# evan-wes/nerf-sandbox

Measured on NVIDIA B200. Metric: train_rays_per_s, higher is better.
Workload: dtype bf16

## Files before the change

nerf_sandbox_b200/csrc/field_tc.cu:

```cuda
#include <cuda.h>
#include <cuda_bf16.h>
#include <cuda_fp16.h>
#include <cstdio>
#include <mutex>
#include "nsb_common.cuh"
#include "tc_ptx.cuh"

namespace nsb {
namespace tc {

constexpr int TILE_M = 128;
constexpr int kStageBytes = 16384;
constexpr int kStages = 4;
constexpr int kActBytes = TILE_M * 256 * 2;
constexpr int kGxBytes = TILE_M * 64 * 2;
constexpr int kSmemAct = 0;
constexpr int kSmemGx = 2 * kActBytes;
constexpr int kSmemRing = kSmemGx + 2 * kGxBytes;
constexpr int kSmemBar = kSmemRing + kStages * kStageBytes;
constexpr int kSmemBias = kSmemBar + 256;
constexpr int kSmemBytes = kSmemBias + 2048;
constexpr int kThreads = 384;
constexpr int kStages2 = 8;
constexpr int kStageBytes2 = kStageBytes / 2;
// ... 823 lines not shown
            tail[layer_bias_ofs(m) + n] = params[d.b_off + n];
    }
    if (m == 0) {
        float* tail = reinterpret_cast<float*>(out + kBiasOfs);
        const LayerDesc ds = layer_desc(9), dc = layer_desc(11);
        for (int i = blockIdx.x * blockDim.x + threadIdx.x; i < 256; i += gridDim.x * blockDim.x) tail[kWsigOfs + i] = params[ds.w_off + i];
        for (int i = blockIdx.x * blockDim.x + threadIdx.x; i < 384; i += gridDim.x * blockDim.x) tail[kWoOfs + i] = params[dc.w_off + i];
        if (blockIdx.x == 0 && threadIdx.x < 4) {
            tail[kBsigOfs + threadIdx.x] = threadIdx.x == 0 ? params[ds.b_off] : 0.f;
            tail[kBoOfs + threadIdx.x] = threadIdx.x < 3 ? params[dc.b_off + threadIdx.x] : 0.f;
        }
    }
}

struct DgradParams {
    const float* d_raw;
    const uint8_t* packed;
    const uint8_t* stash;
    uint8_t* dstash;
    int64_t Q; int64_t num_tiles;
    alignas(64) CUtensorMap tm8;
};

__device__ __forceinline__ uint4 ldg16(const uint8_t* p) { return __ldg(reinterpret_cast<const uint4*>(p)); }
__device__ __forceinline__ float bf16lo(uint32_t w) { return __uint_as_float(w << 16); }
__device__ __forceinline__ float bf16hi(uint32_t w) { return __uint_as_float(w & 0xffff0000u); }

template <int KIND>
__device__ __forceinline__ void dgrad_chunk16(const uint32_t (&v)[16], int c0, uint32_t act, int r, float dsig, float hw0, uint32_t bits16) {
    uint32_t w[8];
#pragma unroll
    for (int j = 0; j < 8; ++j) {
        float a = __uint_as_float(v[2 * j]), b = __uint_as_float(v[2 * j + 1]);
        if (KIND == 1) {
            a = fmaf(dsig, __shfl_sync(0xffffffffu, hw0, (c0 & 16) + 2 * j), a);
            b = fmaf(dsig, __shfl_sync(0xffffffffu, hw0, (c0 & 16) + 2 * j + 1), b);
        }
        w[j] = pack_bf16(a, b);
        if (KIND != 0) w[j] &= relu_mask_word(bits16, j);
    }
    st_chunk(act, (c0 >> 3), r, w[0], w[1], w[2], w[3]);
    st_chunk(act, (c0 >> 3) + 1, r, w[4], w[5], w[6], w[7]);
}
template <int KIND>
__device__ __forceinline__ void dgrad_columns(uint32_t tmem_row, uint32_t act, int r, int lane, const float* __restrict__ tail,
                                              const uint4& mlo, const uint4& mhi, float dsig) {
    float hw0 = KIND == 1 ? __ldg(tail + kWsigOfs + lane) : 0.f;
    const uint32_t mw[8] = {mlo.x, mlo.y, mlo.z, mlo.w, mhi.x, mhi.y, mhi.z, mhi.w};
    uint32_t va[16], vb[16];
    tc_ld16(tmem_row, va);
#pragma unroll
    for (int i = 0; i < 8; ++i) {
        const int c0 = 32 * i;
        float n0 = 0.f;
        if (KIND == 1 && i < 7) n0 = __ldg(tail + kWsigOfs + c0 + 32 + lane);
        tc_wait_ld();
        tc_ld16(tmem_row + (uint32_t)c0 + 16u, vb);
        pin16(va);
        dgrad_chunk16<KIND>(va, c0, act, r, dsig, hw0, mw[i]);
        tc_wait_ld();
        tc_ld16(tmem_row + (uint32_t)(i < 7 ? c0 + 32 : c0), va);
        pin16(vb);
        dgrad_chunk16<KIND>(vb, c0 + 16, act, r, dsig, hw0, mw[i] >> 8);
        hw0 = n0;
    }
}

constexpr int kDgStages = 12;
constexpr int kDgSmemRing = kSmemGx;
static_assert(kDgSmemRing + kDgStages * kStageBytes2 == kSmemBar, "dgrad ring must end at the barrier block");
static_assert(kSmemBar + 8 * (3 * kDgStages + 6) + 4 <= kSmemBytes, "barrier block overflow");
__global__ void __cluster_dims__(2, 1, 1) __launch_bounds__(kThreads, 1) field_dgrad_kernel(const __grid_constant__ DgradParams p) {
    extern __shared__ __align__(128) uint8_t smem[];
    const uint32_t sbase = smem_u32(smem);
    const int warp = threadIdx.x >> 5, lane = threadIdx.x & 31;
    const uint32_t crank = cluster_ctarank();
    const uint32_t bar_full = sbase + kSmemBar, bar_empty = bar_full + 8 * kDgStages, bar_in = bar_empty + 8 * kDgStages,
                   bar_acc = bar_in + 16, bar_pfull = bar_acc + 16, bar_pin = bar_pfull + 8 * kDgStages;
    volatile uint32_t* tmem_slot = reinterpret_cast<volatile uint32_t*>(smem + kSmemBar + 8 * (3 * kDgStages + 6));
    if (threadIdx.x == 0) {
        for (int s = 0; s < kDgStages; ++s) { mbar_init(bar_full + 8 * s, 1); mbar_init(bar_empty + 8 * s, 1); mbar_init(bar_pfull + 8 * s, 1); }
        for (int t = 0; t < 2; ++t) { mbar_init(bar_in + 8 * t, 1); mbar_init(bar_acc + 8 * t, 1); mbar_init(bar_pin + 8 * t, 1); }
        asm volatile("fence.mbarrier_init.release.cluster;" ::: "memory");
    }
    if (warp == 2) {
        asm volatile("tcgen05.alloc.cta_group::2.sync.aligned.shared::cta.b32 [%0], %1;" ::"r"(smem_u32((const void*)tmem_slot)),
                     "r"(kTmemCols)
                     : "memory");
        asm volatile("tcgen05.relinquish_alloc_permit.cta_group::2.sync.aligned;" ::: "memory");
    }
    tc_fence_before();
    __syncthreads();
    cluster_sync_all();
    tc_fence_after();
    const uint32_t tmem_base = *tmem_slot;
    const int64_t num_pairs = (p.num_tiles + 1) / 2;
    const int64_t first_pair = (int64_t)blockIdx.x - crank;
    const int64_t n_iter = first_pair < num_pairs ? (num_pairs - first_pair + gridDim.x - 1) / gridDim.x : 0;
    const float* tail = reinterpret_cast<const float*>(p.packed + kBiasOfs);

    if (warp == 0) {
        {
            uint32_t stage = 0, round = 0;
            for (int64_t it = 0, pair = blockIdx.x; it < n_iter; ++it, pair += gridDim.x) {
                for (int m = 0; m < kNumDgradLayers; ++m) {
                    const uint8_t* src = p.packed + dgrad_layer_ofs(m);
                    const int ns = m == 0 ? 4 : 8;
                    for (int s = 0; s < ns; ++s) {
                        mbar_wait(bar_empty + 8 * stage, (round & 1) ^ 1);
                        if (elect_one()) {
                            if (crank == 0) mbar_expect_tx(bar_full + 8 * stage, kStageBytes);
                            tma_load_rows_to_leader(sbase + kDgSmemRing + stage * kStageBytes2, &p.tm8,
                                                    (dgrad_layer_ofs(m) + (uint32_t)s * kStageBytes + crank * kStageBytes2) >> 8, bar_full + 8 * stage);
                        }
                        __syncwarp();
                        if (++stage == kDgStages) { stage = 0; ++round; }
                    }
                }
            }
        }
    } else if (warp == 1) {
        if (crank == 0 && elect_one()) {
            uint32_t stage = 0, round = 0, use = 0;
            const uint32_t idesc = make_idesc2(256, kFmtBF16, kFmtBF16);
            const uint64_t ahi = desc_hi(2048, 128), bhi = desc_hi(2048, 128);
            const uint32_t ring_lo = (sbase + kDgSmemRing) >> 4;
            for (int64_t it = 0; it < n_iter; ++it) {
                for (int m = 0; m < kNumDgradLayers; ++m, ++use) {
                    const int ns = m == 0 ? 4 : 8;
                    const uint32_t stage0 = stage, round0 = round;
                    for (int t = 0; t < 2; ++t) {
                        mbar_wait(bar_in + 8 * t, use & 1);
                        mbar_wait_cl(bar_pin + 8 * t, use & 1);
                        tc_fence_after();
                        if (t == 1) { stage = stage0; round = round0; }
                        const uint32_t d_tmem = tmem_base + (uint32_t)t * 256u;
                        uint32_t a_lo = (sbase + kSmemAct + t * kActBytes) >> 4;
                        for (int s = 0; s < ns; ++s, a_lo += 512u) {
                            if (t == 0) {
                                mbar_wait(bar_full + 8 * stage, round & 1);
                                tc_fence_after();
                            }
                            const uint32_t b_lo = ring_lo + stage * (kStageBytes2 >> 4);
                            tc_mma2(d_tmem, ahi | (uint64_t)a_lo, bhi | (uint64_t)b_lo, idesc, s > 0 ? 1u : 0u);
                            tc_mma2(d_tmem, ahi | (uint64_t)(a_lo + 256u), bhi | (uint64_t)(b_lo + 256u), idesc, 1u);
                            if (s == ns - 1) tc_commit2(bar_acc + 8 * t);
                            if (t == 1) tc_commit2(bar_empty + 8 * stage);
                            if (++stage == kDgStages) { stage = 0; ++round; }
                        }
                    }
                }
            }
        }
    } else if (warp == 2 || warp == 3) {
        const int t = warp - 2;
        const uint32_t act = sbase + kSmemAct + t * kActBytes;
        named_bar_arrive(1 + t, 160);
        for (int64_t it = 0, pair = blockIdx.x; it < n_iter; ++it, pair += gridDim.x) {
            const int64_t tile = pair * 2 + t;
            uint8_t* ds_tile = tile < p.num_tiles ? p.dstash + (size_t)tile * kDstashTile : nullptr;
            const bool last_pair = it + 1 == n_iter;
            for (int e = 0; e <= kNumDgradLayers; ++e) {
                handoff_wait(t);
                if (lane == 0) {
                    if (e < kNumDgradLayers) arrive_in(crank, bar_in, bar_pin, t);
                    if (ds_tile) {
                        bulk_s2g(ds_tile + (e == 0 ? dstash_ofs(9) : dstash_ofs(8 - (e - 1))), act, e == 0 ? 32768u : 65536u);
                        bulk_commit();
                        bulk_wait_read0();
                    }
                }
                __syncwarp();
                if (!(last_pair && e == kNumDgradLayers)) named_bar_arrive(1 + t, 160);
            }
        }
        if (lane == 0) bulk_wait_all0();
    } else if (warp >= 4) {
        const int t = (warp - 4) >> 2;
        const int r = (int)threadIdx.x - 128 - t * 128;
        const uint32_t act = sbase + kSmemAct + t * kActBytes;
        const uint32_t tmem_row = tmem_base + (uint32_t)t * 256u + ((uint32_t)((warp & 3) * 32) << 16);
        uint32_t use = 0;
        for (int64_t it = 0, pair = blockIdx.x; it < n_iter; ++it, pair += gridDim.x) {
            const int64_t tile = pair * 2 + t;
            const int64_t q = tile * TILE_M + r;
            const bool tile_ok = tile < p.num_tiles;
            const bool valid = tile_ok && q < p.Q;
            const uint8_t* st_tile = p.stash + (size_t)(tile_ok ? tile : 0) * kStashTile;
            const float4 d = valid ? __ldg(reinterpret_cast<const float4*>(p.d_raw) + q) : make_float4(0.f, 0.f, 0.f, 0.f);
            named_bar_sync(1 + t, 160);
            {
                const uint8_t* mrow = st_tile + kStashMask + (size_t)r * 32;
                const uint4 cbits = ldg16(mrow + 8 * 4096);
                const uint32_t cw[4] = {cbits.x, cbits.y, cbits.z, cbits.w};
#pragma unroll
                for (int g = 0; g < 4; ++g) {
                    const float w0 = __ldg(tail + kWoOfs + 32 * g + lane), w1 = __ldg(tail + kWoOfs + 128 + 32 * g + lane),
                                w2 = __ldg(tail + kWoOfs + 256 + 32 * g + lane);
#pragma unroll
                    for (int c8 = 0; c8 < 4; ++c8) {
                        const uint32_t bits16 = cw[g] >> (8 * (c8 >> 1));
                        uint32_t w[4];
#pragma unroll
                        for (int j2 = 0; j2 < 4; ++j2) {
                            const int s0 = c8 * 8 + 2 * j2;
                            const float ga = d.x * __shfl_sync(0xffffffffu, w0, s0) + d.y * __shfl_sync(0xffffffffu, w1, s0) +
                                             d.z * __shfl_sync(0xffffffffu, w2, s0);
                            const float gb = d.x * __shfl_sync(0xffffffffu, w0, s0 + 1) + d.y * __shfl_sync(0xffffffffu, w1, s0 + 1) +
                                             d.z * __shfl_sync(0xffffffffu, w2, s0 + 1);
                            w[j2] = pack_bf16(ga, gb) & relu_mask_word(bits16, 4 * (c8 & 1) + j2);
                        }
                        st_chunk(act, g * 4 + c8, r, w[0], w[1], w[2], w[3]);
                    }
                }
            }
            handoff_signal(t);
            for (int m = 0; m < kNumDgradLayers; ++m, ++use) {
                uint4 mlo = make_uint4(0, 0, 0, 0), mhi = mlo;
                if (m >= 1) {
                    const uint8_t* mrow = st_tile + kStashMask + (size_t)(8 - m) * 4096 + (size_t)r * 32;
                    mlo = ldg16(mrow); mhi = ldg16(mrow + 16);
                }
                mbar_wait(bar_acc + 8 * t, use & 1);
                tc_fence_after();
                named_bar_sync(1 + t, 160);
                if (m == 0) dgrad_columns<0>(tmem_row, act, r, lane, tail, mlo, mhi, d.w);
                else if (m == 1) dgrad_columns<1>(tmem_row, act, r, lane, tail, mlo, mhi, d.w);
                else dgrad_columns<2>(tmem_row, act, r, lane, tail, mlo, mhi, d.w);
                handoff_signal(t);
            }
        }
    }
    tc_fence_before();
    __syncthreads();
    cluster_sync_all();
    if (warp == 2) {
        tc_fence_after();
        asm volatile("tcgen05.dealloc.cta_group::2.sync.aligned.b32 %0, %1;" ::"r"(tmem_base), "r"(kTmemCols) : "memory");
    }
}

struct WgPiece { uint32_t ofs; uint32_t bytes; int from_stash; int dy_half; int head; };
struct WgGroup { int a_piece, b_piece, b_piece2, tmem_col, n; };
enum { HEAD_NONE = 0, HEAD_SIGMA = 1, HEAD_RGB = 2 };
struct WgradJob {
    int n_pieces; WgPiece pieces[4];
    int n_groups; WgGroup groups[4];
    int release_after[4];
    int halves, xcols;
    int64_t w_dst;
    int ldw;
    int ncols_valid;
    int64_t b_dst;
    int64_t head_w_dst, head_b_dst;
    int cta_begin, cta_count;
};
constexpr int kMaxJobs = 16;
struct WgradParams {
    const uint8_t* stash; const uint8_t* dstash; const float* d_raw; float* grads;
    int64_t num_tiles, Q; int num_jobs; int dbg;
    WgradJob jobs[kMaxJobs];
};
constexpr int kWgPiece = 32768;
constexpr int kWgSlots = 6;
constexpr int kWgSmemBar = kWgSlots * kWgPiece;
constexpr int kWgSmemBytes = kWgSmemBar + 256;
constexpr int kWgThreads = 256;

__device__ __forceinline__ uint32_t make_idesc_mn(int N) {
    return (1u << 4) | (kFmtBF16 << 7) | (kFmtBF16 << 10) | (1u << 15) | (1u << 16) | ((uint32_t)(N >> 3) << 17) | ((uint32_t)(TILE_M >> 4) << 24);
}

template <int KIND>
__device__ __forceinline__ void wg_colsum(const uint8_t* img, int nchunks, int w4, int lane, const float4 (&dr)[4], float (&a0)[4][8],
                                          float (&a1)[4][8], float (&a2)[4][8]) {
#pragma unroll
    for (int ii = 0; ii < 4; ++ii) {
        const int c8 = w4 + 4 * ii;
        if (c8 < nchunks) {
#pragma unroll
            for (int rg = 0; rg < 4; ++rg) {
                const uint4 v = *reinterpret_cast<const uint4*>(img + (size_t)c8 * 2048 + (size_t)(rg * 32 + lane) * 16);
                const float x[8] = {bf16lo(v.x), bf16hi(v.x), bf16lo(v.y), bf16hi(v.y), bf16lo(v.z), bf16hi(v.z), bf16lo(v.w), bf16hi(v.w)};
#pragma unroll
                for (int j = 0; j < 8; ++j) {
                    if (KIND == 0) a0[ii][j] += x[j];
                    else if (KIND == 1) a0[ii][j] = fmaf(dr[rg].w, x[j], a0[ii][j]);
                    else {
                        a0[ii][j] = fmaf(dr[rg].x, x[j], a0[ii][j]); a1[ii][j] = fmaf(dr[rg].y, x[j], a1[ii][j]);
                        a2[ii][j] = fmaf(dr[rg].z, x[j], a2[ii][j]);
                    }
                }
            }
        }
    }
}

__global__ void __launch_bounds__(kWgThreads, 1) field_wgrad_kernel(const __grid_constant__ WgradParams p) {
    extern __shared__ __align__(128) uint8_t smem[];
    const uint32_t sbase = smem_u32(smem);
    const int warp = threadIdx.x >> 5, lane = threadIdx.x & 31;
    const uint32_t bar_full = sbase + kWgSmemBar, bar_empty = bar_full + 8 * kWgSlots, bar_done = bar_empty + 8 * kWgSlots;
    volatile uint32_t* tmem_slot = reinterpret_cast<volatile uint32_t*>(smem + kWgSmemBar + 8 * (2 * kWgSlots + 2));
    int ji = 0;
    for (int j = 0; j < p.num_jobs; ++j)
        if ((int)blockIdx.x >= p.jobs[j].cta_begin && (int)blockIdx.x < p.jobs[j].cta_begin + p.jobs[j].cta_count) ji = j;
    const WgradJob& job = p.jobs[ji];
    const int part = (int)blockIdx.x - job.cta_begin;
    if (threadIdx.x == 0) {
        for (int s = 0; s < kWgSlots; ++s) { mbar_init(bar_full + 8 * s, 1); mbar_init(bar_empty + 8 * s, 1 + 4); }
        mbar_init(bar_done, 1);
        asm volatile("fence.mbarrier_init.release.cluster;" ::: "memory");
    }
    if (warp == 2) {
        asm volatile("tcgen05.alloc.cta_group::1.sync.aligned.shared::cta.b32 [%0], %1;" ::"r"(smem_u32((const void*)tmem_slot)),
                     "r"(kTmemCols)
                     : "memory");
        asm volatile("tcgen05.relinquish_alloc_permit.cta_group::1.sync.aligned;" ::: "memory");
    }
    tc_fence_before();
    __syncthreads();
    tc_fence_after();
    const uint32_t tmem_base = *tmem_slot;
    int64_t my_tiles = 0;
    for (int64_t tile = part; tile < p.num_tiles; tile += job.cta_count) ++my_tiles;

    if (warp == 0) {
        uint32_t slot = 0, round = 0;
        for (int64_t tile = part; tile < p.num_tiles; tile += job.cta_count) {
            for (int i = 0; i < job.n_pieces; ++i) {
                const WgPiece& pc = job.pieces[i];
                const int64_t pt = p.num_tiles - 1 - tile;
                const uint8_t* src = pc.from_stash ? p.stash + (size_t)pt * kStashTile + pc.ofs : p.dstash + (size_t)pt * kDstashTile + pc.ofs;
                mbar_wait(bar_empty + 8 * slot, (round & 1) ^ 1);
                if (elect_one()) {
                    mbar_expect_tx(bar_full + 8 * slot, pc.bytes);
                    bulk_g2s(sbase + slot * kWgPiece, src, pc.bytes, bar_full + 8 * slot);
                }
                __syncwarp();
                if (++slot == kWgSlots) { slot = 0; ++round; }
            }
        }
    } else if (warp == 1) {
        if (elect_one()) {
            uint32_t slot = 0, round = 0;
            const uint64_t mnhi = desc_hi(128, 2048);
            bool first = true;
            long long w_full = 0; const long long t_begin = clock64();
            for (int64_t tile = part; tile < p.num_tiles; tile += job.cta_count) {
                uint32_t pslot[4], pround[4];
                for (int i = 0; i < job.n_pieces; ++i) { pslot[i] = slot; pround[i] = round; if (++slot == kWgSlots) { slot = 0; ++round; } }
                uint32_t ready = 0;
                for (int g = 0; g < job.n_groups; ++g) {
                    const WgGroup& gr = job.groups[g];
                    const long long tw0 = clock64();
                    if (!(ready >> gr.a_piece & 1)) { mbar_wait(bar_full + 8 * pslot[gr.a_piece], pround[gr.a_piece] & 1); ready |= 1u << gr.a_piece; }
                    if (!(ready >> gr.b_piece & 1)) { mbar_wait(bar_full + 8 * pslot[gr.b_piece], pround[gr.b_piece] & 1); ready |= 1u << gr.b_piece; }
                    if (gr.b_piece2 >= 0 && !(ready >> gr.b_piece2 & 1)) {
                        mbar_wait(bar_full + 8 * pslot[gr.b_piece2], pround[gr.b_piece2] & 1); ready |= 1u << gr.b_piece2;
                    }
                    w_full += clock64() - tw0;
                    tc_fence_after();
                    const uint32_t a_lo = (sbase + pslot[gr.a_piece] * kWgPiece) >> 4, b_lo = (sbase + pslot[gr.b_piece] * kWgPiece) >> 4;
                    const uint32_t idesc = make_idesc_mn(gr.n);
#pragma unroll
                    for (int ks = 0; ks < 8; ++ks)
                        tc_mma(tmem_base + (uint32_t)gr.tmem_col, mnhi | (uint64_t)(a_lo + ks * 16), mnhi | (uint64_t)(b_lo + ks * 16), idesc,
                               (!first || ks > 0) ? 1u : 0u);
                    for (int i = 0; i < job.n_pieces; ++i)
                        if (job.release_after[i] == g) tc_commit(bar_empty + 8 * pslot[i]);
                }
                for (int i = 0; i < job.n_pieces; ++i)
                    if (job.release_after[i] < 0) { mbar_wait(bar_full + 8 * pslot[i], pround[i] & 1); mbar_arrive(bar_empty + 8 * pslot[i]); }
                first = false;
            }
            tc_commit(bar_done);
            if (p.dbg && (part == 0)) printf("wgrad job %d (%d CTAs, %lld tiles): mma thread waited for pieces %lld of %lld cycles\n", ji, job.cta_count, (long long)my_tiles, w_full, clock64() - t_begin);
        }
    } else if (warp >= 4) {
        const int w4 = warp - 4;
        float bsum[2][4][8];
        float hacc[3][4][8];
        float dsum[4] = {0.f, 0.f, 0.f, 0.f};
#pragma unroll
        for (int i = 0; i < 4; ++i)
#pragma unroll
            for (int j = 0; j < 8; ++j) { bsum[0][i][j] = bsum[1][i][j] = 0.f; hacc[0][i][j] = hacc[1][i][j] = hacc[2][i][j] = 0.f; }
        const bool want_bias = job.b_dst >= 0;
        int job_head = HEAD_NONE;
        for (int i = 0; i < job.n_pieces; ++i) if (job.pieces[i].head) job_head = job.pieces[i].head;
        auto load_dr = [&](int64_t tile, float4 (&dr)[4]) {
#pragma unroll
            for (int rg = 0; rg < 4; ++rg) {
                const int64_t q = (p.num_tiles - 1 - tile) * TILE_M + rg * 32 + lane;
                dr[rg] = (tile < p.num_tiles && q < p.Q) ? __ldg(reinterpret_cast<const float4*>(p.d_raw) + q) : make_float4(0.f, 0.f, 0.f, 0.f);
            }
        };
        {
            uint32_t slot = 0, round = 0;
            float4 dr[4], dr_next[4];
            if (job_head) load_dr(part, dr_next);
            for (int64_t tile = part; tile < p.num_tiles; tile += job.cta_count) {
                if (job_head) {
#pragma unroll
                    for (int rg = 0; rg < 4; ++rg) dr[rg] = dr_next[rg];
                    load_dr(tile + job.cta_count, dr_next);
                    if (w4 == 0) {
#pragma unroll
                        for (int rg = 0; rg < 4; ++rg) { dsum[0] += dr[rg].x; dsum[1] += dr[rg].y; dsum[2] += dr[rg].z; dsum[3] += dr[rg].w; }
                    }
                }
                int xhalf = 0;
                for (int i = 0; i < job.n_pieces; ++i) {
                    const WgPiece& pc = job.pieces[i];
                    mbar_wait(bar_full + 8 * slot, round & 1);
                    const uint8_t* img = smem + slot * kWgPiece;
                    const int nchunks = (int)(pc.bytes >> 11);
                    if (pc.dy_half == 0 && want_bias) wg_colsum<0>(img, nchunks, w4, lane, dr, bsum[0], bsum[0], bsum[0]);
                    else if (pc.dy_half == 1 && want_bias) wg_colsum<0>(img, nchunks, w4, lane, dr, bsum[1], bsum[1], bsum[1]);
                    if (pc.head == HEAD_SIGMA) {
                        if (xhalf == 0) wg_colsum<1>(img, nchunks, w4, lane, dr, hacc[0], hacc[0], hacc[0]);
                        else wg_colsum<1>(img, nchunks, w4, lane, dr, hacc[1], hacc[1], hacc[1]);
                        ++xhalf;
                    } else if (pc.head == HEAD_RGB) {
                        wg_colsum<2>(img, nchunks, w4, lane, dr, hacc[0], hacc[1], hacc[2]);
                    }
                    __syncwarp();
                    if (lane == 0) mbar_arrive(bar_empty + 8 * slot);
                    if (++slot == kWgSlots) { slot = 0; ++round; }
                }
            }
        }
        if (my_tiles > 0) {
            if (want_bias) {
#pragma unroll
                for (int a = 0; a < 2; ++a)
#pragma unroll
                    for (int ii = 0; ii < 4; ++ii)
#pragma unroll
                        for (int j = 0; j < 8; ++j) {
                            const float sum = warp_sum(bsum[a][ii][j]);
                            if (lane == 0 && a < job.halves) atomicAdd(p.grads + job.b_dst + a * 128 + (w4 + 4 * ii) * 8 + j, sum);
                        }
            }
            if (job_head == HEAD_SIGMA) {
#pragma unroll
                for (int a = 0; a < 2; ++a)
#pragma unroll
                    for (int ii = 0; ii < 4; ++ii)
#pragma unroll
                        for (int j = 0; j < 8; ++j) {
                            const float sum = warp_sum(hacc[a][ii][j]);
                            if (lane == 0) atomicAdd(p.grads + job.head_w_dst + a * 128 + (w4 + 4 * ii) * 8 + j, sum);
                        }
                if (w4 == 0) { const float sd = warp_sum(dsum[3]); if (lane == 0) atomicAdd(p.grads + job.head_b_dst, sd); }
            } else if (job_head == HEAD_RGB) {
#pragma unroll
                for (int ch = 0; ch < 3; ++ch)
#pragma unroll
                    for (int ii = 0; ii < 4; ++ii)
#pragma unroll
                        for (int j = 0; j < 8; ++j) {
                            const float sum = warp_sum(hacc[ch][ii][j]);
                            if (lane == 0) atomicAdd(p.grads + job.head_w_dst + ch * 128 + (w4 + 4 * ii) * 8 + j, sum);
                        }
                if (w4 == 0) {
                    const float a0 = warp_sum(dsum[0]), a1 = warp_sum(dsum[1]), a2 = warp_sum(dsum[2]);
                    if (lane == 0) { atomicAdd(p.grads + job.head_b_dst, a0); atomicAdd(p.grads + job.head_b_dst + 1, a1); atomicAdd(p.grads + job.head_b_dst + 2, a2); }
                }
            }
            if (job.n_groups > 0) {
                mbar_wait(bar_done, 0);
                tc_fence_after();
                for (int h = 0; h < job.halves; ++h) {
                    const int n = h * 128 + w4 * 32 + lane;
                    const uint32_t trow = tmem_base + (uint32_t)h * 256u + ((uint32_t)(w4 * 32) << 16);
                    for (int c0 = 0; c0 < job.xcols; c0 += 32) {
                        uint32_t v[32];
                        tc_ld32(trow + (uint32_t)c0, v);
                        tc_wait_ld();
                        float* dst = p.grads + job.w_dst + (int64_t)n * job.ldw + c0;
#pragma unroll
                        for (int j = 0; j < 32; ++j)
                            if (c0 + j < job.ncols_valid) atomicAdd(dst + j, __uint_as_float(v[j]));
                    }
                }
            }
        }
    }
    tc_fence_before();
    __syncthreads();
    if (warp == 2) {
        tc_fence_after();
        asm volatile("tcgen05.dealloc.cta_group::1.sync.aligned.b32 %0, %1;" ::"r"(tmem_base), "r"(kTmemCols) : "memory");
    }
}

struct DinputParams {
    const uint8_t* packed; const uint8_t* dstash;
    float* d_enc_pos; float* d_enc_dir;
    int64_t Q, num_tiles;
};
constexpr int kDiSlab = 16384;
constexpr int kDiStages = 4;
constexpr int kDiSlabs = 10;
constexpr int kDiSmemRing = kDinImgBytes;
constexpr int kDiSmemOut = kDiSmemRing + kDiStages * kDiSlab;
constexpr int kDiOutFloats = TILE_M * (kPosDim + kDirDim);
constexpr int kDiSmemBar = kDiSmemOut + kDiOutFloats * 4;
constexpr int kDiSmemBytes = kDiSmemBar + 256;
constexpr int kDiThreads = 256;
constexpr uint32_t kDiTmemCols = 256;
static_assert(kDiSmemBytes <= 227 * 1024, "dinput shared memory");
__host__ __device__ inline size_t dinput_slab_ofs(int s) {
    return s < 4 ? dstash_ofs(0) + (size_t)s * kDiSlab : (s < 8 ? dstash_ofs(4) + (size_t)(s - 4) * kDiSlab : dstash_ofs(9) + (size_t)(s - 8) * kDiSlab);
}

__global__ void __launch_bounds__(kDiThreads, 1) field_dinput_kernel(const __grid_constant__ DinputParams p) {
    extern __shared__ __align__(128) uint8_t smem[];
    const uint32_t sbase = smem_u32(smem);
    const int warp = threadIdx.x >> 5;
    const uint32_t bar_full = sbase + kDiSmemBar, bar_empty = bar_full + 8 * kDiStages, bar_acc = bar_empty + 8 * kDiStages,
                   bar_free = bar_acc + 16, bar_b = bar_free + 16;
    volatile uint32_t* tmem_slot = reinterpret_cast<volatile uint32_t*>(smem + kDiSmemBar + 8 * (2 * kDiStages + 5));
    if (threadIdx.x == 0) {
        for (int s = 0; s < kDiStages; ++s) { mbar_init(bar_full + 8 * s, 1); mbar_init(bar_empty + 8 * s, 1); }
        for (int a = 0; a < 2; ++a) { mbar_init(bar_acc + 8 * a, 1); mbar_init(bar_free + 8 * a, 128); }
        mbar_init(bar_b, 1);
        asm volatile("fence.mbarrier_init.release.cluster;" ::: "memory");
    }
    if (warp == 2) {
        asm volatile("tcgen05.alloc.cta_group::1.sync.aligned.shared::cta.b32 [%0], %1;" ::"r"(smem_u32((const void*)tmem_slot)),
                     "r"(kDiTmemCols)
                     : "memory");
        asm volatile("tcgen05.relinquish_alloc_permit.cta_group::1.sync.aligned;" ::: "memory");
    }
    tc_fence_before();
    __syncthreads();
    tc_fence_after();
    const uint32_t tmem_base = *tmem_slot;

    if (warp == 0) {
        if (elect_one()) {
            mbar_expect_tx(bar_b, kDinImgBytes);
            bulk_g2s(sbase, p.packed + kDinImgOfs, kDinImgBytes, bar_b);
            uint32_t stage = 0, round = 0;
            for (int64_t tile = blockIdx.x; tile < p.num_tiles; tile += gridDim.x) {
                const uint8_t* ds = p.dstash + (size_t)tile * kDstashTile;
                for (int s = 0; s < kDiSlabs; ++s) {
                    mbar_wait(bar_empty + 8 * stage, (round & 1) ^ 1);
                    mbar_expect_tx(bar_full + 8 * stage, kDiSlab);
                    bulk_g2s(sbase + kDiSmemRing + stage * kDiSlab, ds + dinput_slab_ofs(s), kDiSlab, bar_full + 8 * stage);
                    if (++stage == kDiStages) { stage = 0; ++round; }
                }
            }
        }
    } else if (warp == 1) {
        if (elect_one()) {
            constexpr uint32_t idesc_base = (1u << 4) | (1u << 7) | (1u << 10) | ((uint32_t)(TILE_M >> 4) << 24);
            constexpr uint32_t idesc_x = idesc_base | ((uint32_t)(64 >> 3) << 17), idesc_d = idesc_base | ((uint32_t)(32 >> 3) << 17);
            const uint64_t ahi = desc_hi(2048, 128), bhi_x = desc_hi(64 * 16, 128), bhi_d = desc_hi(32 * 16, 128);
            mbar_wait(bar_b, 0);
            uint32_t stage = 0, round = 0, it = 0;
            for (int64_t tile = blockIdx.x; tile < p.num_tiles; tile += gridDim.x, ++it) {
                const uint32_t acc = it & 1;
                mbar_wait(bar_free + 8 * acc, ((it >> 1) & 1) ^ 1);
                tc_fence_after();
                const uint32_t d_x = tmem_base + acc * 128, d_d = d_x + 64;
                for (int s = 0; s < kDiSlabs; ++s) {
                    mbar_wait(bar_full + 8 * stage, round & 1);
                    tc_fence_after();
                    const uint32_t a0 = sbase + kDiSmemRing + stage * kDiSlab;
#pragma unroll
                    for (int j = 0; j < 4; ++j) {
                        const uint64_t ad = desc_at(ahi, a0 + j * 4096);
                        if (s < 8) {
                            const uint32_t k0 = (uint32_t)(s & 3) * 64 + j * 16;
                            const uint32_t b = sbase + (s < 4 ? kDinPos0 : kDinPos4) + (k0 >> 3) * 1024;
                            tc_mma(d_x, ad, desc_at(bhi_x, b), idesc_x, (s == 0 && j == 0) ? 0u : 1u);
                        } else {
                            const uint32_t k0 = (uint32_t)(s - 8) * 64 + j * 16;
                            tc_mma(d_d, ad, desc_at(bhi_d, sbase + kDinDir + (k0 >> 3) * 512), idesc_d, (s == 8 && j == 0) ? 0u : 1u);
                        }
                    }
                    tc_commit(bar_empty + 8 * stage);
                    if (++stage == kDiStages) { stage = 0; ++round; }
                }
                tc_commit(bar_acc + 8 * acc);
            }
        }
    } else if (warp >= 4) {
        const int r = (int)threadIdx.x - 128;
        float* out_x = reinterpret_cast<float*>(smem + kDiSmemOut);
        float* out_d = out_x + TILE_M * kPosDim;
        uint32_t it = 0;
        for (int64_t tile = blockIdx.x; tile < p.num_tiles; tile += gridDim.x, ++it) {
            const uint32_t acc = it & 1;
            mbar_wait(bar_acc + 8 * acc, (it >> 1) & 1);
            tc_fence_after();
            const uint32_t trow = tmem_base + acc * 128 + ((uint32_t)((warp & 3) * 32) << 16);
#pragma unroll 1
            for (int c = 0; c < 6; ++c) {
                uint32_t v[16];
                tc_ld16(trow + 16 * c, v);
                tc_wait_ld();
                pin16(v);
#pragma unroll
                for (int j = 0; j < 16; ++j) {
                    const int col = 16 * c + j;
                    if (col < kPosDim) out_x[r * kPosDim + col] = __uint_as_float(v[j]);
                    else if (col >= 64 && col < 64 + kDirDim) out_d[r * kDirDim + col - 64] = __uint_as_float(v[j]);
                }
            }
            tc_fence_before();
            mbar_arrive(bar_free + 8 * acc);
            named_bar_sync(1, 128);
            const int64_t rows = p.Q - tile * TILE_M < TILE_M ? p.Q - tile * TILE_M : TILE_M;
            if (p.d_enc_pos) {
                float* dst = p.d_enc_pos + tile * TILE_M * kPosDim;
                for (int i = r; i < rows * kPosDim; i += 128) dst[i] = out_x[i];
            }
            if (p.d_enc_dir) {
                float* dst = p.d_enc_dir + tile * TILE_M * kDirDim;
                for (int i = r; i < rows * kDirDim; i += 128) dst[i] = out_d[i];
            }
            named_bar_sync(1, 128);
        }
    }
    tc_fence_before();
    __syncthreads();
    if (warp == 2) {
        tc_fence_after();
        asm volatile("tcgen05.dealloc.cta_group::1.sync.aligned.b32 %0, %1;" ::"r"(tmem_base), "r"(kDiTmemCols) : "memory");
    }
}

__device__ __forceinline__ void pack_tc_dinput(const float* __restrict__ params, uint8_t* __restrict__ out) {
    const LayerDesc d0 = layer_desc(0), d4 = layer_desc(4), dc = layer_desc(10);
    for (int idx = blockIdx.x * blockDim.x + threadIdx.x; idx < 2 * 32 * 64 + 16 * 32; idx += gridDim.x * blockDim.x) {
        int img = idx >> 11, rem = idx & 2047;
        if (img > 2) img = 2;
        if (img == 2) rem = idx - 2 * 2048;
        const int rows = img < 2 ? 64 : 32, n = rem % rows, k8 = rem / rows;
        const LayerDesc& d = img == 0 ? d0 : (img == 1 ? d4 : dc);
        const int col = img == 0 ? n : kHidden + n, n_true = img < 2 ? kPosDim : kDirDim;
        float x[8];
#pragma unroll
        for (int j = 0; j < 8; ++j) x[j] = n < n_true ? params[d.w_off + (int64_t)(8 * k8 + j) * d.K + col] : 0.f;
        const uint32_t base = img == 0 ? kDinPos0 : (img == 1 ? kDinPos4 : kDinDir);
        *reinterpret_cast<uint4*>(out + kDinImgOfs + base + (size_t)(k8 * rows + n) * 16) =
            make_uint4(pack_bf16(x[0], x[1]), pack_bf16(x[2], x[3]), pack_bf16(x[4], x[5]), pack_bf16(x[6], x[7]));
    }
}

__device__ __forceinline__ void pack_tc_transposed(const float* __restrict__ params, uint8_t* __restrict__ out, int m) {
    {
        const int pl = m == 0 ? 10 : (m == 1 ? 8 : 9 - m);
        const LayerDesc d = layer_desc(pl);
        const int Nout = d.N;
        __nv_bfloat16* img = reinterpret_cast<__nv_bfloat16*>(out + dgrad_layer_ofs(m));
        for (int idx = blockIdx.x * blockDim.x + threadIdx.x; idx < (Nout >> 3) * 256; idx += gridDim.x * blockDim.x) {
            const int n8 = idx >> 8, j = idx & 255;
            const float* col = params + d.w_off + (int64_t)(8 * n8) * d.K + j;
            uint32_t w[4];
#pragma unroll
            for (int q = 0; q < 4; ++q) w[q] = pack_bf16(col[(int64_t)(2 * q) * d.K], col[(int64_t)(2 * q + 1) * d.K]);
            reinterpret_cast<uint4*>(img)[(((size_t)(n8 >> 2) * 2 + (j >> 7)) * 4 + (n8 & 3)) * 128 + (j & 127)] = make_uint4(w[0], w[1], w[2], w[3]);
        }
    }
}
struct PackBatch { const float* params[4]; uint8_t* out[4]; uint64_t* counter; };
__global__ void pack_tc_kernel(const PackBatch b) {
    if (b.counter && blockIdx.x == 0 && blockIdx.y == 0 && blockIdx.z == 0 && threadIdx.x == 0) *b.counter += 1;
    const float* params = b.params[blockIdx.z];
    uint8_t* out = b.out[blockIdx.z];
    if (blockIdx.y < kNumMmaLayers) pack_tc_forward<0>(params, out, blockIdx.y);
    else if (blockIdx.y < kNumMmaLayers + kNumDgradLayers) pack_tc_transposed(params, out, blockIdx.y - kNumMmaLayers);
    else if (blockIdx.y == kNumMmaLayers + kNumDgradLayers) pack_tc_dinput(params, out);
    else if (blockIdx.y < 2 * kNumMmaLayers + kNumDgradLayers + 1) pack_tc_forward<1>(params, out, blockIdx.y - kNumMmaLayers - kNumDgradLayers - 1);
    else pack_tc_forward<2>(params, out, blockIdx.y - 2 * kNumMmaLayers - kNumDgradLayers - 1);
}

}

size_t tc_packed_bytes() { return align_up(tc::kPackedTcBytes, 256); }

size_t tc_workspace_bytes(int64_t Q, int stash) {
    const int64_t tiles = cdiv(Q, tc::TILE_M);
    return 256 + (stash ? (size_t)tiles * (tc::kStashTile + tc::kDstashTile) : 0);
}
size_t tc_stash_tile_bytes() { return tc::kStashTile; }
static inline uint8_t* ws_stash(void* ws) { return reinterpret_cast<uint8_t*>(ws) + 256; }
static inline uint8_t* ws_dstash(void* ws, int64_t Q) { return ws_stash(ws) + (size_t)cdiv(Q, tc::TILE_M) * tc::kStashTile; }

int tc_pack(const float* const* params, void* const* packed_bf16, int n_nets, bool train_only, cudaStream_t st) {
    tc::PackBatch b{};
    for (int i = 0; i < n_nets; ++i) { b.params[i] = params[i]; b.out[i] = reinterpret_cast<uint8_t*>(packed_bf16[i]); }
    b.counter = g_pack_counter;
    const int ny = train_only ? tc::kNumMmaLayers + tc::kNumDgradLayers + 1 : 3 * tc::kNumMmaLayers + tc::kNumDgradLayers + 1;
    tc::pack_tc_kernel<<<dim3(32, ny, n_nets), 256, 0, st>>>(b);
    NSB_LAUNCH_CHECK("pack_tc_kernel");
    return NSB_OK;
}

int check_arch() {
    static int ok = -1;
    if (ok < 0) {
        int dev = 0, major = 0;
        cudaGetDevice(&dev);
        cudaDeviceGetAttribute(&major, cudaDevAttrComputeCapabilityMajor, dev);
        ok = major == 10 ? 1 : 0;
    }
    return ok ? NSB_OK : NSB_E_ARCH;
}

struct PackedMaps { const void* ptr; CUtensorMap tm8, tm4; };
static int packed_maps(const void* packed, CUtensorMap* tm8, CUtensorMap* tm4) {
    typedef CUresult (*EncodeFn)(CUtensorMap*, CUtensorMapDataType, cuuint32_t, void*, const cuuint64_t*, const cuuint64_t*, const cuuint32_t*,
                                 const cuuint32_t*, CUtensorMapInterleave, CUtensorMapSwizzle, CUtensorMapL2promotion, CUtensorMapFloatOOBfill);
    static std::mutex mu;
    static EncodeFn encode = nullptr;
    static PackedMaps cache[16];
    static int n_cached = 0, next = 0;
    std::lock_guard<std::mutex> lock(mu);
    for (int i = 0; i < n_cached; ++i)
        if (cache[i].ptr == packed) { *tm8 = cache[i].tm8; if (tm4) *tm4 = cache[i].tm4; return NSB_OK; }
    if (!encode) {
        void* fn = nullptr;
        cudaDriverEntryPointQueryResult q;
        if (cudaGetDriverEntryPoint("cuTensorMapEncodeTiled", &fn, cudaEnableDefault, &q) != cudaSuccess || !fn)
            return check_launch("cudaGetDriverEntryPoint(cuTensorMapEncodeTiled)");
        encode = reinterpret_cast<EncodeFn>(fn);
    }
    PackedMaps m{};
    m.ptr = packed;
    const cuuint64_t dims[2] = {256, tc::kPackedTcBytes / 256};
    const cuuint64_t strides[1] = {256};
    const cuuint32_t estr[2] = {1, 1};
    for (int k = 0; k < 2; ++k) {
        const cuuint32_t box[2] = {256, k == 0 ? 32u : 16u};
        if (encode(k == 0 ? &m.tm8 : &m.tm4, CU_TENSOR_MAP_DATA_TYPE_UINT8, 2, const_cast<void*>(packed), dims, strides, box, estr,
                   CU_TENSOR_MAP_INTERLEAVE_NONE, CU_TENSOR_MAP_SWIZZLE_NONE, CU_TENSOR_MAP_L2_PROMOTION_L2_256B,
                   CU_TENSOR_MAP_FLOAT_OOB_FILL_NONE) != CUDA_SUCCESS) {
            snprintf(g_cuda_err, sizeof(g_cuda_err), "cuTensorMapEncodeTiled failed for the packed weight buffer");
            return NSB_E_CUDA;
        }
    }
    cache[next] = m; next = (next + 1) % 16; if (n_cached < 16) ++n_cached;
    *tm8 = m.tm8; if (tm4) *tm4 = m.tm4;
    return NSB_OK;
}

template <bool FROM_ENC>
static int launch_fwd(tc::FwdParams& p, cudaStream_t st) {
    NSB_TRY(check_arch());
    static bool attr_set = false;
    if (!attr_set) {
        if (cudaFuncSetAttribute(tc::field_fwd_kernel<FROM_ENC, false>, cudaFuncAttributeMaxDynamicSharedMemorySize, tc::kSmemBytes) != cudaSuccess ||
            cudaFuncSetAttribute(tc::field_fwd_kernel<FROM_ENC, true>, cudaFuncAttributeMaxDynamicSharedMemorySize, tc::kSmemBytes) != cudaSuccess)
            return check_launch("cudaFuncSetAttribute(field_fwd_kernel)");
        attr_set = true;
    }
    p.num_tiles = cdiv(p.Q, tc::TILE_M);
    NSB_TRY(packed_maps(p.packed, &p.tm8, &p.tm4));
    const int64_t pairs = (p.num_tiles + 1) / 2;
    int grid = (int)(pairs < num_sms() ? pairs : num_sms());
    grid = (grid + 1) / 2 * 2;
    if (grid > num_sms()) grid -= 2;
    if (p.stash) tc::field_fwd_kernel<FROM_ENC, true><<<grid, tc::kThreads, tc::kSmemBytes, st>>>(p);
    else tc::field_fwd_kernel<FROM_ENC, false><<<grid, tc::kThreads, tc::kSmemBytes, st>>>(p);
    NSB_LAUNCH_CHECK("field_fwd_kernel");
    return NSB_OK;
}

template <bool FROM_ENC>
static int launch_fwd_split(tc::FwdParams& p, cudaStream_t st) {
    NSB_TRY(check_arch());
    static bool attr_set = false;
    if (!attr_set) {
        if (cudaFuncSetAttribute(tc::field_fwd_split_kernel<FROM_ENC>, cudaFuncAttributeMaxDynamicSharedMemorySize, tc::kSmemBytes) != cudaSuccess)
            return check_launch("cudaFuncSetAttribute(field_fwd_split_kernel)");
        attr_set = true;
    }
    p.num_tiles = cdiv(p.Q, tc::TILE_M);
    NSB_TRY(packed_maps(p.packed, &p.tm8, &p.tm4));
    const int64_t pairs = (p.num_tiles + 1) / 2;
    const int64_t max_pairs = num_sms() / 2;
    const int grid = 2 * (int)(pairs < max_pairs ? pairs : max_pairs);
    tc::field_fwd_split_kernel<FROM_ENC><<<grid, tc::kThreads, tc::kSmemBytes, st>>>(p);
    NSB_LAUNCH_CHECK("field_fwd_split_kernel");
    return NSB_OK;
}

int tc_field_fwd_rays_split(const float* rays_o, const float* rays_d, const float* z, const float* ray_norm, const float* viewdirs,
                            const void* packed, float* raw, int64_t B, int N, cudaStream_t st) {
    tc::FwdParams p{};
    p.rays_o = rays_o; p.rays_d = rays_d; p.z = z; p.ray_norm = ray_norm; p.viewdirs = viewdirs;
    p.packed = reinterpret_cast<const uint8_t*>(packed); p.raw = raw;
    p.Q = B * (int64_t)N; p.N = N;
    return launch_fwd_split<false>(p, st);
}
int tc_field_fwd_enc_split(const float* enc_pos, const float* enc_dir, const void* packed, float* raw, int64_t Q, cudaStream_t st) {
    tc::FwdParams p{};
    p.enc_pos = enc_pos; p.enc_dir = enc_dir;
    p.packed = reinterpret_cast<const uint8_t*>(packed); p.raw = raw;
    p.Q = Q; p.N = 1;
    return launch_fwd_split<true>(p, st);
}

int tc_field_fwd_rays(const float* rays_o, const float* rays_d, const float* z, const float* ray_norm, const float* viewdirs,
                      const void* packed, float* raw, void* ws, int64_t B, int N, int stash, cudaStream_t st) {
    tc::FwdParams p{};
    p.rays_o = rays_o; p.rays_d = rays_d; p.z = z; p.ray_norm = ray_norm; p.viewdirs = viewdirs;
    p.packed = reinterpret_cast<const uint8_t*>(packed); p.raw = raw;
    p.stash = stash ? ws_stash(ws) : nullptr;
    p.Q = B * (int64_t)N; p.N = N;
    return launch_fwd<false>(p, st);
}

int tc_field_fwd_enc(const float* enc_pos, const float* enc_dir, const void* packed, float* raw, void* ws, int64_t Q,
                     int stash, cudaStream_t st) {
    tc::FwdParams p{};
    p.enc_pos = enc_pos; p.enc_dir = enc_dir;
    p.packed = reinterpret_cast<const uint8_t*>(packed); p.raw = raw;
    p.stash = stash ? ws_stash(ws) : nullptr;
    p.Q = Q; p.N = 1;
    return launch_fwd<true>(p, st);
}

int tc_field_bwd(const float* d_raw, const void* packed, float* grads, float* d_enc_pos, float* d_enc_dir, void* ws, int64_t Q,
                 cudaStream_t st) {
    NSB_TRY(check_arch());
    static bool attr_set = false;
    if (!attr_set) {
        if (cudaFuncSetAttribute(tc::field_dgrad_kernel, cudaFuncAttributeMaxDynamicSharedMemorySize, tc::kSmemBytes) != cudaSuccess ||
            cudaFuncSetAttribute(tc::field_wgrad_kernel, cudaFuncAttributeMaxDynamicSharedMemorySize, tc::kWgSmemBytes) != cudaSuccess ||
            cudaFuncSetAttribute(tc::field_dinput_kernel, cudaFuncAttributeMaxDynamicSharedMemorySize, tc::kDiSmemBytes) != cudaSuccess)
            return check_launch("cudaFuncSetAttribute(bwd kernels)");
        attr_set = true;
    }
    const int64_t tiles = cdiv(Q, tc::TILE_M);
    const int64_t pairs = (tiles + 1) / 2;
    tc::DgradParams dp{};
    dp.d_raw = d_raw; dp.packed = reinterpret_cast<const uint8_t*>(packed); dp.stash = ws_stash(ws); dp.dstash = ws_dstash(ws, Q);
    dp.Q = Q; dp.num_tiles = tiles;
    NSB_TRY(packed_maps(packed, &dp.tm8, nullptr));
    int dgrid = (int)(pairs < num_sms() ? pairs : num_sms());
    dgrid = (dgrid + 1) / 2 * 2;
    if (dgrid > num_sms()) dgrid -= 2;
    tc::field_dgrad_kernel<<<dgrid, tc::kThreads, tc::kSmemBytes, st>>>(dp);
    NSB_LAUNCH_CHECK("field_dgrad_kernel");
    if (d_enc_pos || d_enc_dir) {
        tc::DinputParams ip{};
        ip.packed = reinterpret_cast<const uint8_t*>(packed); ip.dstash = ws_dstash(ws, Q);
        ip.d_enc_pos = d_enc_pos; ip.d_enc_dir = d_enc_dir; ip.Q = Q; ip.num_tiles = tiles;
        const int igrid = (int)(tiles < num_sms() ? tiles : num_sms());
        tc::field_dinput_kernel<<<igrid, tc::kDiThreads, tc::kDiSmemBytes, st>>>(ip);
        NSB_LAUNCH_CHECK("field_dinput_kernel");
    }
    if (!grads) return NSB_OK;

    tc::WgradParams wp{};
    wp.stash = ws_stash(ws); wp.dstash = ws_dstash(ws, Q); wp.d_raw = d_raw; wp.grads = grads; wp.num_tiles = tiles; wp.Q = Q;
    int nj = 0;
    auto add = [&](int k, size_t x_ofs, int xcols, int pl, int col0, int valid, bool bias, int head) {
        const LayerDesc d = layer_desc(pl);
        tc::WgradJob& j = wp.jobs[nj++];
        j = tc::WgradJob{};
        const int halves = k == 9 ? 1 : 2;
        const uint32_t dy = (uint32_t)tc::dstash_ofs(k);
        const uint32_t xb = (uint32_t)xcols * 256u;
        auto piece = [&](uint32_t ofs, uint32_t bytes, int from_stash, int dy_half, int hd) {
            j.pieces[j.n_pieces] = tc::WgPiece{ofs, bytes, from_stash, dy_half, hd}; j.release_after[j.n_pieces] = -1; return j.n_pieces++;
        };
        auto group = [&](int a, int b, int col, int n) {
            j.groups[j.n_groups] = tc::WgGroup{a, b, -1, col, n}; j.release_after[a] = j.n_groups; j.release_after[b] = j.n_groups; ++j.n_groups;
        };
        if (xcols == 256) {
            const int b0 = piece((uint32_t)x_ofs, 32768, 1, -1, head), b1 = piece((uint32_t)x_ofs + 32768, 32768, 1, -1, head);
            const int a0 = piece(dy, 32768, 0, 0, 0);
            group(a0, b0, 0, 256);
            if (halves == 2) { const int a1 = piece(dy + 32768, 32768, 0, 1, 0); group(a1, b0, 256, 256); }
            for (int g = 0; g < j.n_groups; ++g) j.groups[g].b_piece2 = b1;
            j.release_after[b1] = j.n_groups - 1;
        } else {
            const int a0 = piece(dy, 32768, 0, 0, 0);
            const int b0 = piece((uint32_t)x_ofs, xb, 1, -1, head);
            group(a0, b0, 0, xcols);
            if (halves == 2) { const int a1 = piece(dy + 32768, 32768, 0, 1, 0); group(a1, b0, 256, xcols); }
        }
        j.halves = halves; j.xcols = xcols;
        j.w_dst = d.w_off + col0; j.ldw = d.K; j.ncols_valid = valid; j.b_dst = bias ? d.b_off : -1;
        if (head == tc::HEAD_SIGMA) { const LayerDesc ds = layer_desc(9); j.head_w_dst = ds.w_off; j.head_b_dst = ds.b_off; }
    };
    add(0, tc::kStashGx, 64, 0, 0, 63, true, 0);
    for (int l = 1; l <= 7; ++l) {
        add(l, tc::kStashH + (size_t)(l - 1) * 65536, 256, l, 0, 256, true, 0);
        if (l == 4) add(4, tc::kStashGx, 64, 4, 256, 63, false, 0);
    }
    add(8, tc::kStashH + 7 * 65536, 256, 8, 0, 256, true, tc::HEAD_SIGMA);
    add(9, tc::kStashFeat, 256, 10, 0, 256, true, 0);
    add(9, tc::kStashGd, 32, 10, 256, 27, false, 0);
    {
        tc::WgradJob& j = wp.jobs[nj++];
        j = tc::WgradJob{};
        j.pieces[0] = tc::WgPiece{(uint32_t)tc::kStashC, 32768, 1, -1, tc::HEAD_RGB}; j.release_after[0] = -1; j.n_pieces = 1;
        const LayerDesc dc = layer_desc(11);
        j.head_w_dst = dc.w_off; j.head_b_dst = dc.b_off; j.b_dst = -1;
    }
    wp.num_jobs = nj;
    wp.dbg = getenv("NSB_WG_DBG") != nullptr;
    const int total = num_sms();
    double cost[tc::kMaxJobs];
    for (int i = 0; i < nj; ++i) {
        const tc::WgradJob& j = wp.jobs[i];
        if (j.n_groups == 0) cost[i] = 1750;
        else if (j.xcols == 256) cost[i] = j.halves == 2 ? 5600 : 3100;
        else cost[i] = j.xcols == 64 ? 3750 : 2100;
        if (j.head_w_dst && j.n_groups) cost[i] += 100;
        wp.jobs[i].cta_count = 1;
    }
    for (int used = nj; used < total; ++used) {
        int worst = -1; double worst_t = -1;
        for (int i = 0; i < nj; ++i) {
            if ((int64_t)wp.jobs[i].cta_count >= tiles) continue;
            const double t = cost[i] * (double)cdiv(tiles, wp.jobs[i].cta_count);
            if (t > worst_t) { worst_t = t; worst = i; }
        }
        if (worst < 0) break;
        ++wp.jobs[worst].cta_count;
    }
    int begin = 0;
    for (int i = 0; i < nj; ++i) { wp.jobs[i].cta_begin = begin; begin += wp.jobs[i].cta_count; }
    tc::field_wgrad_kernel<<<begin, tc::kWgThreads, tc::kWgSmemBytes, st>>>(wp);
    NSB_LAUNCH_CHECK("field_wgrad_kernel");
    return NSB_OK;
}

int tc_debug_layer(const float* rays_o, const float* rays_d, const float* z, const float* ray_norm, const float* viewdirs,
                   const void* packed, float* raw, float* dbg, int layer, int64_t B, int N, cudaStream_t st) {
    tc::FwdParams p{};
    if (layer < 0) {
        p.cyc = reinterpret_cast<unsigned long long*>(dbg);
        if (layer == -2) p.stash = reinterpret_cast<uint8_t*>(dbg) + 256;
        dbg = nullptr;
    }
    p.rays_o = rays_o; p.rays_d = rays_d; p.z = z; p.ray_norm = ray_norm; p.viewdirs = viewdirs;
    p.packed = reinterpret_cast<const uint8_t*>(packed); p.raw = raw; p.dbg = dbg; p.dbg_layer = layer;
    p.Q = B * (int64_t)N; p.N = N;
    return launch_fwd<false>(p, st);
}

}
```

Measured before the change: 816,400.

## Stage TMEM weight-gradient flush through shared memory with vectorized float4 atomics

The epilogue of the weight-gradient kernel now moves each 32x32 TMEM block through a padded, double-buffered shared-memory tile and overlaps the next TMEM load with the current flush. Each warp then issues coalesced float4 atomicAdds row by row instead of scalar atomics along a strided per-thread row, which cuts the number and scatter of global atomics. The host-side CTA split heuristic now adds a per-job flush cost term so the CTA allocation accounts for this epilogue. The debug print is deferred to a single thread after the barrier. The staging reuses shared memory at offset zero, which assumes the ring contents are no longer needed at this point.

```diff
diff --git a/nerf_sandbox_b200/csrc/field_tc.cu b/nerf_sandbox_b200/csrc/field_tc.cu
--- a/nerf_sandbox_b200/csrc/field_tc.cu
+++ b/nerf_sandbox_b200/csrc/field_tc.cu
@@ -1149,6 +1149,7 @@
     const int warp = threadIdx.x >> 5, lane = threadIdx.x & 31;
     const uint32_t bar_full = sbase + kWgSmemBar, bar_empty = bar_full + 8 * kWgSlots, bar_done = bar_empty + 8 * kWgSlots;
     volatile uint32_t* tmem_slot = reinterpret_cast<volatile uint32_t*>(smem + kWgSmemBar + 8 * (2 * kWgSlots + 2));
+    long long* dbg_cyc = reinterpret_cast<long long*>(smem + kWgSmemBar + 128);
     int ji = 0;
     for (int j = 0; j < p.num_jobs; ++j)
         if ((int)blockIdx.x >= p.jobs[j].cta_begin && (int)blockIdx.x < p.jobs[j].cta_begin + p.jobs[j].cta_count) ji = j;
@@ -1222,7 +1223,7 @@
                 first = false;
             }
             tc_commit(bar_done);
-            if (p.dbg && (part == 0)) printf("wgrad job %d (%d CTAs, %lld tiles): mma thread waited for pieces %lld of %lld cycles\n", ji, job.cta_count, (long long)my_tiles, w_full, clock64() - t_begin);
+            if (p.dbg && part == 0) { dbg_cyc[0] = w_full; dbg_cyc[1] = clock64() - t_begin; }
         }
     } else if (warp >= 4) {
         const int w4 = warp - 4;
@@ -1318,25 +1319,56 @@
             }
             if (job.n_groups > 0) {
                 mbar_wait(bar_done, 0);
+                named_bar_sync(1, 128);
                 tc_fence_after();
-                for (int h = 0; h < job.halves; ++h) {
-                    const int n = h * 128 + w4 * 32 + lane;
-                    const uint32_t trow = tmem_base + (uint32_t)h * 256u + ((uint32_t)(w4 * 32) << 16);
-                    for (int c0 = 0; c0 < job.xcols; c0 += 32) {
-                        uint32_t v[32];
-                        tc_ld32(trow + (uint32_t)c0, v);
-                        tc_wait_ld();
-                        float* dst = p.grads + job.w_dst + (int64_t)n * job.ldw + c0;
-#pragma unroll
-                        for (int j = 0; j < 32; ++j)
-                            if (c0 + j < job.ncols_valid) atomicAdd(dst + j, __uint_as_float(v[j]));
-                    }
-                }
+                const long long tf0 = clock64();
+                constexpr int kStg = 36;
+                const uint32_t stg = sbase + (uint32_t)w4 * (2u * 32u * kStg * 4u);
+                const int nc = job.xcols >> 5, nb = job.halves * nc;
+                const bool vec = ((job.ldw | job.w_dst | job.ncols_valid) & 3) == 0 && (reinterpret_cast<uintptr_t>(p.grads) & 15) == 0;
+                auto taddr = [&](int b) { return tmem_base + (uint32_t)(b / nc) * 256u + (uint32_t)(b % nc) * 32u + ((uint32_t)(w4 * 32) << 16); };
+                uint32_t v[32];
+                tc_ld32(taddr(0), v);
+                for (int b = 0; b < nb; ++b) {
+                    const uint32_t buf = stg + (uint32_t)(b & 1) * (32u * kStg * 4u);
+                    tc_wait_ld();
+#pragma unroll
+                    for (int q = 0; q < 8; ++q)
+                        asm volatile("st.shared.v4.b32 [%0], {%1, %2, %3, %4};" ::"r"(buf + (uint32_t)(lane * kStg + 4 * q) * 4u), "r"(v[4 * q]),
+                                     "r"(v[4 * q + 1]), "r"(v[4 * q + 2]), "r"(v[4 * q + 3])
+                                     : "memory");
+                    __syncwarp();
+                    if (b + 1 < nb) tc_ld32(taddr(b + 1), v);
+                    const int c0 = (b % nc) * 32;
+                    float* dst = p.grads + job.w_dst + (int64_t)((b / nc) * 128 + w4 * 32) * job.ldw + c0;
+                    if (vec) {
+                        const int cq = (lane & 7) * 4;
+#pragma unroll
+                        for (int rr = 0; rr < 32; rr += 4) {
+                            const int r = rr + (lane >> 3);
+                            float4 s;
+                            asm volatile("ld.shared.v4.f32 {%0, %1, %2, %3}, [%4];" : "=f"(s.x), "=f"(s.y), "=f"(s.z), "=f"(s.w)
+                                         : "r"(buf + (uint32_t)(r * kStg + cq) * 4u) : "memory");
+                            if (c0 + cq < job.ncols_valid) atomicAdd(reinterpret_cast<float4*>(dst + (int64_t)r * job.ldw + cq), s);
+                        }
+                    } else {
+#pragma unroll 8
+                        for (int r = 0; r < 32; ++r) {
+                            float s;
+                            asm volatile("ld.shared.f32 %0, [%1];" : "=f"(s) : "r"(buf + (uint32_t)(r * kStg + lane) * 4u) : "memory");
+                            if (c0 + lane < job.ncols_valid) atomicAdd(dst + (int64_t)r * job.ldw + lane, s);
+                        }
+                    }
+                }
+                if (p.dbg && part == 0 && w4 == 0 && lane == 0) dbg_cyc[2] = clock64() - tf0;
             }
         }
     }
     tc_fence_before();
     __syncthreads();
+    if (p.dbg && part == 0 && threadIdx.x == 128)
+        printf("wgrad job %d (%d CTAs, %lld tiles): mma thread waited for pieces %lld of %lld cycles; flush %lld cycles\n", ji, job.cta_count,
+               (long long)my_tiles, dbg_cyc[0], dbg_cyc[1], my_tiles > 0 && job.n_groups > 0 ? dbg_cyc[2] : 0ll);
     if (warp == 2) {
         tc_fence_after();
         asm volatile("tcgen05.dealloc.cta_group::1.sync.aligned.b32 %0, %1;" ::"r"(tmem_base), "r"(kTmemCols) : "memory");
@@ -1758,20 +1790,23 @@
     wp.num_jobs = nj;
     wp.dbg = getenv("NSB_WG_DBG") != nullptr;
     const int total = num_sms();
-    double cost[tc::kMaxJobs];
+    const bool grads_v4 = (reinterpret_cast<uintptr_t>(grads) & 15) == 0;
+    double cost[tc::kMaxJobs], flush[tc::kMaxJobs];
     for (int i = 0; i < nj; ++i) {
         const tc::WgradJob& j = wp.jobs[i];
         if (j.n_groups == 0) cost[i] = 1750;
         else if (j.xcols == 256) cost[i] = j.halves == 2 ? 5600 : 3100;
         else cost[i] = j.xcols == 64 ? 3750 : 2100;
         if (j.head_w_dst && j.n_groups) cost[i] += 100;
+        const bool v4 = grads_v4 && ((j.ldw | j.w_dst | j.ncols_valid) & 3) == 0;
+        flush[i] = j.n_groups ? (v4 ? 0.23 : 0.8) * (double)(j.halves * 128 * j.xcols) : 0.0;
         wp.jobs[i].cta_count = 1;
     }
     for (int used = nj; used < total; ++used) {
         int worst = -1; double worst_t = -1;
         for (int i = 0; i < nj; ++i) {
             if ((int64_t)wp.jobs[i].cta_count >= tiles) continue;
-            const double t = cost[i] * (double)cdiv(tiles, wp.jobs[i].cta_count);
+            const double t = cost[i] * (double)cdiv(tiles, wp.jobs[i].cta_count) + flush[i];
             if (t > worst_t) { worst_t = t; worst = i; }
         }
         if (worst < 0) break;
```

After: 847,200 (median of 6 runs). 3.8% higher.
